# M2-TE/noetic-slam

Measured on AMD Instinct MI355X. Metric: scans/sec TSDF integration (128x1024 pts, 5 cm voxel), higher is better.
Workload: dtype f64+f32; 1 GPU; C1/M1 ouster_os1_128_1024x10_synthetic_5cm; global_batch=64, scans_per_gpu_batch=64, pipelined_batches=2, semantics=vdbfusion_f64, parallelism=single, front_end=two walks (k_count + k_place)

## Files before the change

### noetic-slam_amd/csrc/tsdf_capi.cpp

```cpp
#include <hip/hip_runtime.h>

#include <algorithm>
#include <array>
#include <atomic>
#include <cmath>
#include <cstdarg>
#include <cstddef>
#include <cstdio>
#include <cstdlib>
#include <cstring>
#include <numeric>
#include <chrono>
#include <condition_variable>
#include <functional>
#include <mutex>
#include <string>
#include <thread>
#include <utility>
#include <vector>

#include "../../include/tsdf_hip.h"
#include "../../include/tsdf_hip_raycast.h"
#include "../../include/tsdf_hip_sample.h"
#include "../../include/tsdf_mc_tables.h"
// ... 168 lines not shown
    H h = nullptr;
    HipHandle() = default;
    HipHandle(const HipHandle&) = delete;
    HipHandle& operator=(const HipHandle&) = delete;
    ~HipHandle() { if (h) (void)KILL(h); }
    hipError_t create() { return MAKE(&h, FLAGS); }
    operator H() const { return h; }
};
using Event = HipHandle<hipEvent_t, hipEventCreateWithFlags, hipEventDisableTiming, hipEventDestroy>;
using Stream = HipHandle<hipStream_t, hipStreamCreateWithFlags, hipStreamNonBlocking, hipStreamDestroy>;


struct Capacity {
    uint64_t max_bricks = 0, cap = 0;
    uint32_t max_active = 0;
    DevBuf<uint64_t> keys, brick_keys;
    DevBuf<uint32_t> slots, touched, cell[2];
    DevBuf<float> sdf, weight;
    DevBuf<uint4> active[2], active_ord[2], cagg[2];
};

struct Lane {
    DevBuf<uint32_t> pair, blk_n, plan, spn, ord_hist, act;
    DevBuf<uint4> blk, fb;
    DevBuf<uint2> smp;
    DevBuf<uint64_t> mg_ekey;
    DevBuf<uint32_t> mg_eidx, mg_bcnt, mg_bst, mg_bscan;
    DevBuf<float> mg_xyz, mg_w;
};

struct ScanRing {
    static constexpr int N = 16;
    PinBuf<ScanRec> host;
    DevBuf<ScanRec> dev;
    const ScanRec* host_dev = nullptr;
    PinBuf<unsigned long long> done;
    unsigned long long* done_dev = nullptr;
    Event ev[N];
    uint64_t next = 0;

    hipError_t create() {
        hipError_t e = host.alloc((size_t)N * (MAX_BATCH + 1));
        if (e == hipSuccess) e = dev.alloc((size_t)N * (MAX_BATCH + 1));
        void* dp = nullptr;
        if (e == hipSuccess) e = hipHostGetDevicePointer(&dp, host, 0);
        host_dev = static_cast<const ScanRec*>(dp);
// ... 5 lines not shown
        return e;
    }
};

}

struct tsdf_ctx {
    tsdf_params p{};
    int device = -1;
    Stream stream;
    RayConst R{};
    Table T{};
    Pool Pl{};
    Work W2[2]{};
    MgBufs mg[2];
    DevBuf<Globals> G;
    uint64_t max_points = 0;
    uint32_t max_batch = 0;
    CtxPlan plan;
    uint32_t max_fb = 0, max_smp = 0, max_spn = 0;
    int small_ns = 5;
    uint32_t count_wide = 512;
    bool count_paired = false;
    PinBuf<float> h_stage[2];
    Event stage_done[2];
    int stage_cur = 0;
    Stream bst[2];
    Capacity K;
    Lane lane[2];
    DevBuf<float> stage2[2];
    Event ev_main;
    Event ev_compact[2];
    hipEvent_t ev_integ[2] = {nullptr, nullptr};
    BatchDesc pend{};
    int pend_stage = 0;
    int last_stage = 1;
    uint64_t stage_reader[2] = {~0ull, ~0ull};
    Event stage_ev[2];
    ScanRing ring;
    HostTiming ht;
    uint64_t batch_id = 0;
    uint64_t n_scans = 0, n_batches = 0, n_points_in = 0;
    EventTimer* timer = nullptr;
    std::string err;
    struct Logged { uint64_t id; const float* xyz; BatchDesc D; };
    std::vector<Logged> log;
// ... 86 lines not shown
        if (rc) return rc;
    }
    D.s[0].blk = 0;
    for (uint32_t s = 0; s < D.n_scans; s++)
        D.s[s + 1].blk = D.s[s].blk + (D.s[s + 1].off - D.s[s].off + RPB - 1) / RPB;
    D.n_blocks = D.s[D.n_scans].blk;
    if (D.n_blocks > c->plan.max_blocks)
        return fail(c, TSDF_EINVAL, "batch needs %u workgroups > %u", D.n_blocks, c->plan.max_blocks);
    const int par = (int)(c->batch_id & 1);
    c->ht.lap(HT_PRE);
    const bool cross = c->p.pipeline != 0, lean = c->p.pipeline == 2;
    hipStream_t st = c->bst[cross ? par : 0];
    Table T = c->T;
    T.cell = c->K.cell[par];
    const Work& W = c->W2[par];
    const bool prev = cross && c->batch_id > 0;
    EventTimer* tm = c->timer;
    if (tm) tm->cur_batch = c->batch_id;
    if (c->metrics) c->metrics_info.push_back({c->batch_id, D.n_scans, D.s[D.n_scans].off});
    if (hipStreamQuery(c->stream) != hipSuccess) {
        HIPCHK(c, hipEventRecord(c->ev_main, c->stream));
        HIPCHK(c, hipStreamWaitEvent(st, c->ev_main, 0));
    }
    if (prev) HIPCHK(c, hipStreamWaitEvent(st, c->ev_compact[par ^ 1], 0));
    c->ht.lap(HT_WAITS);
    ScanRing& ring = c->ring;
    const uint64_t seq = ring.next++;
    const int slot = (int)(seq % ScanRing::N);
    if (const int rc = ring_wait(c, seq)) return rc;
    c->ht.lap(HT_RING_WAIT);
    const size_t at = (size_t)slot * (MAX_BATCH + 1);
    ScanRec* ds = ring.dev + at;
    std::memcpy(ring.host + at, D.s, (D.n_scans + 1) * sizeof(ScanRec));
    c->ht.lap(HT_RING_COPY);
    HIPCHK(c, launch_upload(ring.host_dev + at, ds, (uint32_t)((D.n_scans + 1) * sizeof(ScanRec)),
                            ring.done_dev, seq + 1, st));
    c->ht.lap(HT_UPLOAD);
    const BatchRef B{D.n_scans, D.n_blocks, ds};
    RayConst R = c->R;
    const float* d_rays = d_xyz;
    if (c->merged && D.n_blocks) {
        HIPCHK(c, launch_mg_prepass(d_xyz, B, D.n_blocks, D.s[D.n_scans].off, c->R, c->mg[par],
                                    &c->G->ctr[par].ovf, st));
        d_rays = c->mg[par].xyz_out;
        R.ray_w = c->mg[par].w_out;
    }
    const bool small = !c->plan.fused && D.n_scans <= (uint32_t)c->small_ns;
    const int k_front = c->plan.fused ? KIND_WALK : KIND_COUNT;
    const int k_back = c->plan.fused ? KIND_SPANS : KIND_PLACE;
    auto kt = [&](int kind) { return tm && !c->plan.fused && tm->want(kind) ? tm->timing(kind) : KTime{}; };
    if (D.n_blocks) {
        if (tm && c->plan.fused) tm->begin(k_front, st);
        if (c->R.sec_on) HIPCHK(c, launch_sector_flags(d_rays, B, R, W, c->G, par, st));
        if (c->plan.fused) HIPCHK(c, launch_walk(d_rays, B, R, T, W, c->G, par, c->plan.nstep, st));
        else HIPCHK(c, launch_count(d_rays, B, R, T, W, c->G, par, st, kt(KIND_COUNT),
                                    !c->R.sec_on && D.n_blocks <= c->count_wide,
                                    !c->R.sec_on && c->count_paired));
        c->ht.lap(HT_FRONT);
        if (tm && c->plan.fused) tm->next(k_front, KIND_COMPACT, st);
        HIPCHK(c, launch_compact(B, T, W, c->G, par, c->plan.fused, st, kt(KIND_COMPACT)));
        c->ht.lap(HT_COMPACT);
// ... 2 lines not shown
    if (prev && lean) HIPCHK(c, hipStreamWaitEvent(st, c->ev_integ[par ^ 1], 0));
    if (D.n_blocks) {
        if (tm && c->plan.fused) tm->next(KIND_COMPACT, k_back, st);
        if (c->plan.fused) HIPCHK(c, launch_spans(B, c->R, T, W, c->G, par, c->plan.nstep, st));
        else HIPCHK(c, launch_place(d_rays, B, R, T, W, c->G, par, st, kt(KIND_PLACE)));
        c->ht.lap(HT_BACK);
        if (tm && c->plan.fused) tm->end(k_back, st);
    }
    if (lean) HIPCHK(c, hipEventRecord(c->ev_compact[par], st));
    if (prev && !lean) HIPCHK(c, hipStreamWaitEvent(st, c->ev_integ[par ^ 1], 0));
    if (D.n_blocks) {
        if (tm && c->plan.fused) tm->begin(KIND_INTEGRATE, st);
        if (small) {
            HIPCHK(c, launch_integrate_small(B, c->R, T, W, c->Pl, c->G, par, st, kt(KIND_INTEGRATE)));
        } else {
            Work Wi = W;
            Wi.active = W.active_ord;
            HIPCHK(c, launch_integrate(B, c->R, T, Wi, c->Pl, c->G, par, c->plan.fused, c->max_batch > 64, st,
                                       kt(KIND_INTEGRATE)));
        }
        if (tm && c->plan.fused) tm->end(KIND_INTEGRATE, st);
        c->ht.lap(HT_INTEGRATE);
    }
    HIPCHK(c, launch_finish(c->G, par, (uint32_t)c->batch_id, st));
    if (cross) {
        HIPCHK(c, hipEventRecord(ring.ev[slot], st));
        c->ev_integ[par] = ring.ev[slot];
    }
    if (c->can_grow) c->log.push_back({c->batch_id, d_xyz, D});
    for (int k = 0; k < 2; k++)
        if (d_xyz == c->stage2[k]) {
            c->stage_reader[k] = c->batch_id;
            HIPCHK(c, hipEventRecord(c->stage_ev[k], st));
        }
    c->ht.lap(HT_FINISH);
    c->ht.n++;
    c->batch_id++;
    c->n_batches++;
    c->n_scans += D.n_scans;
    if (tm && tm->pending.size() > 8192) {
        HIPCHK(c, hipStreamSynchronize(c->bst[0]));
        HIPCHK(c, hipStreamSynchronize(c->bst[1]));
        tm->harvest();
    }
    return TSDF_OK;
}

// ... 238 lines not shown

static int emit_metrics(tsdf_ctx* c) {
    if (!c->metrics) return TSDF_OK;
    if (c->timer) c->timer->harvest();
    const uint64_t end = c->batch_id;
    if (end == c->metrics_next) return TSDF_OK;
    std::vector<BatchRecord> ring(METRIC_RING);
    HIPCHK(c, hipMemcpy(ring.data(), c->G->ring, sizeof(BatchRecord) * METRIC_RING,
                        hipMemcpyDeviceToHost));
    size_t ti = 0;
    for (uint64_t b = std::max<uint64_t>(c->metrics_next, end > METRIC_RING ? end - METRIC_RING : 0);
         b < end; b++) {
        const BatchRecord& r = ring[b % METRIC_RING];
        if (r.batch_id != (uint32_t)b) continue;
        uint32_t scans = 0;
        uint64_t points = 0;
        for (auto& i : c->metrics_info)
            if (i.id == b) { scans = i.scans; points = i.points; }
        const double bytes = 12.0 * (double)r.rays + 16.0 * (double)r.vox;
        fprintf(c->metrics,
                "{\"batch\": %llu, \"scans\": %u, \"points\": %llu, \"rays\": %llu, \"pairs\": %llu, "
                "\"voxel_updates\": %llu, \"dirty_voxels\": %llu, \"active_bricks\": %u, "
                "\"new_bricks\": %u, \"bricks\": %u, \"overflow\": %u, \"committed\": %s, "
                "\"algorithmic_bytes\": %.0f",
                (unsigned long long)b, scans, (unsigned long long)points,
                (unsigned long long)r.rays, (unsigned long long)r.pairs, (unsigned long long)r.vox,
                (unsigned long long)r.dirty, r.n_active, r.n_new,
                std::min<uint32_t>(r.pool_count, c->T.max_bricks), r.ovf,
                r.committed ? "true" : "false", bytes);
        const std::array<double, KIND_N>* ms = nullptr;
        if (c->timer) {
            auto& bm = c->timer->batch_ms;
            while (ti < bm.size() && bm[ti].first < b) ti++;
            if (ti < bm.size() && bm[ti].first == b) ms = &bm[ti].second;
        }
        if (ms) {
            double path = 0;
            for (int k = 0; k < KIND_N; k++) path += (*ms)[k];
            if (c->plan.fused)
                fprintf(c->metrics,
                        ", \"kernel_ms\": {\"walk\": %.5f, \"compact\": %.5f, \"spans\": %.5f, "
                        "\"integrate\": %.5f}",
                        (*ms)[KIND_WALK], (*ms)[KIND_COMPACT], (*ms)[KIND_SPANS], (*ms)[KIND_INTEGRATE]);
            else
                fprintf(c->metrics,
                        ", \"kernel_ms\": {\"count\": %.5f, \"compact\": %.5f, \"place\": %.5f, "
                        "\"integrate\": %.5f}",
                        (*ms)[KIND_COUNT], (*ms)[KIND_COMPACT], (*ms)[KIND_PLACE], (*ms)[KIND_INTEGRATE]);
            fprintf(c->metrics, ", \"path_ms\": %.5f, \"gbs\": %.2f", path,
                    path > 0 ? bytes / (path * 1e-3) / 1e9 : 0.0);
        }
        fprintf(c->metrics, "}\n");
// ... 204 lines not shown
    c->plan = ctx_plan(*p, PlanConsts{RPB, MAX_BATCH, WLK_THREADS, SPAN, VOX_LIMIT});
    if (!c->plan.refusal.empty()) return fail(c, TSDF_EINVAL, "%s", c->plan.refusal.c_str());
    c->R = ray_const(*p, c->plan.band_vox);
    c->merged = plan_merged(*p);
    c->idx_rule = p->n_sectors > 1 && p->sector_rule == TSDF_SECTOR_RULE_INDEX;
    c->max_points = p->max_points;
    c->max_batch = p->max_batch;
    c->max_fb = c->plan.max_fb;
    c->max_smp = c->plan.max_smp;
    c->max_spn = c->plan.max_spn;

    for (int q = 0; q < 2; q++) {
        Lane& L = c->lane[q];
        HIPCHK(c, L.pair.alloc(c->plan.fused ? 4 : c->plan.slots));
        HIPCHK(c, L.blk.alloc((size_t)c->plan.max_blocks * 2 * HCAP));
        HIPCHK(c, L.blk_n.alloc((size_t)c->plan.max_blocks * 2));
        HIPCHK(c, L.plan.alloc((size_t)c->plan.max_blocks * 2 * PLAN_STRIDE));
        HIPCHK(c, L.fb.alloc(c->max_fb));
        HIPCHK(c, L.smp.alloc_bytes((size_t)c->max_smp * smp_bytes(c->R.sem)));
        HIPCHK(c, L.spn.alloc(c->max_spn));
        HIPCHK(c, L.ord_hist.alloc(2 * 64 * 32));
        HIPCHK(c, hipMemset(L.ord_hist, 0, 2 * 64 * 32 * sizeof(uint32_t)));
        HIPCHK(c, L.act.alloc(c->plan.max_blocks));
        HIPCHK(c, c->stage2[q].alloc(c->plan.batch_points * 3));
        if (c->merged) {
            const uint64_t n = c->plan.batch_points, nb = mg_buckets_max(n);
            HIPCHK(c, L.mg_ekey.alloc(n));
            HIPCHK(c, L.mg_eidx.alloc(n));
            HIPCHK(c, L.mg_bcnt.alloc(MG_REPLICAS * nb));
            HIPCHK(c, hipMemset(L.mg_bcnt, 0, 4 * MG_REPLICAS * nb));
            HIPCHK(c, L.mg_bst.alloc(nb + 1));
            HIPCHK(c, L.mg_bscan.alloc(nb));
            HIPCHK(c, L.mg_xyz.alloc(n * 3));
            HIPCHK(c, L.mg_w.alloc(n));
        }
    }
    HIPCHK(c, c->G.alloc(1));
    if (const char* e = std::getenv("TSDF_SMALL_NS")) c->small_ns = std::max(0, std::min(8, std::atoi(e)));
    if (const char* e = std::getenv("TSDF_COUNT_WIDE")) c->count_wide = (uint32_t)std::max(0, std::atoi(e));
    if (const char* e = std::getenv("TSDF_COUNT_PAIRED")) c->count_paired = std::atoi(e) != 0;
    int nt = 4;
    if (const char* e = std::getenv("TSDF_PACK_THREADS")) nt = std::max(1, std::atoi(e));
    nt = std::min<int>(nt, (int)std::max(1u, std::thread::hardware_concurrency()));
    if (nt > 1) {
        try {
            c->pack = new PackPool(nt - 1);
        } catch (...) {
            c->pack = nullptr;
        }
    }
    HIPCHK(c, c->ring.create());
    HIPCHK(c, hipMemsetAsync(c->G, 0, sizeof(Globals), c->stream));
    Capacity K;
    if (const int rc = alloc_capacity(c, p->max_bricks, K)) return rc;
    HIPCHK(c, launch_fill(K.sdf, c->R.bg, p->max_bricks * BRICK_VOX, c->stream));
    HIPCHK(c, hipMemsetAsync(K.weight, 0, p->max_bricks * BRICK_VOX * sizeof(float), c->stream));
    c->K = std::move(K);
    set_views(c);
    for (int i = 0; i < 2; i++) {
        HIPCHK(c, c->h_stage[i].alloc(c->max_points * 3));
        HIPCHK(c, c->stage_done[i].create());
    }
    c->can_grow = p->max_bricks_hard == 0 || p->max_bricks_hard > p->max_bricks;
// ... 1617 lines not shown
```

### noetic-slam_amd/csrc/tsdf_device.h

```cpp
#pragma once
#include <hip/hip_ext.h>
#include <hip/hip_runtime.h>
#include <stdint.h>

namespace tsdf {

constexpr uint64_t EMPTY_KEY = ~0ull;
constexpr uint32_t UNASSIGNED = 0xFFFFFFFFu;
constexpr uint32_t INVALID_SLOT = 0xFFFFFFFEu;
constexpr uint32_t NO_PAIR = 0xFFFFFFFFu;
constexpr int BRICK_VOX = 512;
constexpr int BRICK_COORD_BIAS = 1 << 20;
constexpr int VOX_LIMIT = 1 << 23;
constexpr int MAX_DDA_STEPS = 1 << 20;
constexpr int MAX_BATCH = 512;
#ifndef TSDF_RPB
#define TSDF_RPB 1024
#endif
#ifndef TSDF_HCAP
#define TSDF_HCAP 2048
#endif
constexpr int RPB = TSDF_RPB;
constexpr int HCAP = TSDF_HCAP;
constexpr int LDS_PROBES = 64;
// ... 60 lines not shown
    if (!R.sec_on) return true;
    const float a = pseudo_angle(dx, dy);
    return R.sec_wrap ? (a >= R.sec_lo || a < R.sec_hi) : (a >= R.sec_lo && a < R.sec_hi);
}

struct ScanRec {
    uint32_t off, blk;
    float ox, oy, oz;
    float zx;
    double odx, ody, odz;
    float zy, zz;
    uint32_t xoff, pad;
};
static_assert(sizeof(ScanRec) == 64, "ScanRec layout");
struct BatchDesc {
    uint32_t n_scans;
    uint32_t n_blocks;
    ScanRec s[MAX_BATCH + 1];
};
struct BatchRef {
    uint32_t n_scans;
    uint32_t n_blocks;
    const ScanRec* __restrict__ s;
};

struct Table {
    uint64_t* keys;
    uint32_t* slots;
    uint32_t* touched;
    uint32_t* cell;
    uint64_t* brick_keys;
    uint64_t mask;
    uint32_t max_bricks;
    uint32_t cell_stride;
};

struct Pool {
    float* sdf;
    float* weight;
};

struct Work {
    uint32_t* pair;
    uint4* blk;
    uint32_t* blk_n;
    uint32_t* plan;
// ... 28 lines not shown
        return make_uint2(v.x, v.y);
    } else {
        return W.smp[i];
    }
}

struct Counters {
    uint32_t n_active;
    uint32_t cursor;
    uint32_t n_fb;
    uint32_t ovf;
    uint32_t n_new;
    uint32_t n_act;
    uint32_t pad1[2];
    unsigned long long n_vox[8];
    unsigned long long n_rays[8];
    unsigned long long n_pairs[8];
    unsigned long long n_dirty[8];
};

constexpr uint32_t METRIC_RING = 256;
struct BatchRecord {
    uint32_t batch_id, n_active, n_new, ovf;
    uint32_t committed, pool_count, pad[2];
    unsigned long long rays, pairs, vox, dirty;
};

struct Globals {
    uint32_t pool_count;
    uint32_t overflow;
    uint32_t failed;
    uint32_t retry;
    uint32_t fail_id;
    uint32_t pad[3];
    Counters ctr[2];
    unsigned long long tot_vox[8];
    unsigned long long tot_rays[8];
    unsigned long long tot_pairs[8];
    unsigned long long tot_dirty[8];
    Counters last;
    BatchRecord ring[METRIC_RING];
};

enum KernelKind {
    KIND_COUNT = 0, KIND_COMPACT = 1, KIND_PLACE = 2, KIND_INTEGRATE = 3,
    KIND_WALK = 4, KIND_SPANS = 5,
    KIND_N = 6
// ... 1 lines not shown

struct KTime {
    hipEvent_t start = nullptr, stop = nullptr;
};
template <typename... KArgs, typename... Args>
inline void tlaunch(void (*kern)(KArgs...), dim3 grid, dim3 block, hipStream_t st, hipEvent_t e0,
                    hipEvent_t e1, Args... args) {
    if (!e0 && !e1) {
        kern<<<grid, block, 0, st>>>(args...);
        return;
    }
    hipExtLaunchKernelGGL(kern, grid, block, 0, st, e0, e1, 0, args...);
}

struct KernelTimer {
    virtual void begin(int kind, hipStream_t st) = 0;
    virtual void end(int kind, hipStream_t st) = 0;
    virtual ~KernelTimer() {}
};

hipError_t launch_count(const float* d_xyz, const BatchRef& D, const RayConst& R, const Table& T,
                        const Work& Wk, Globals* G, int parity, hipStream_t st, const KTime& kt = {},
                        bool wide = false, bool paired = false);
#ifndef TSDF_CMP_CHUNK
#define TSDF_CMP_CHUNK 1024
#endif
constexpr uint32_t CMP_CHUNK = TSDF_CMP_CHUNK;
inline uint64_t compact_chunks(uint64_t cap) { return (cap + CMP_CHUNK - 1) / CMP_CHUNK; }
hipError_t launch_sector_flags(const float* d_xyz, const BatchRef& D, const RayConst& R,
                               const Work& Wk, Globals* G, int parity, hipStream_t st);
hipError_t launch_compact(const BatchRef& D, const Table& T, const Work& Wk, Globals* G,
                          int parity, bool fused, hipStream_t st, const KTime& kt = {});
hipError_t launch_walk(const float* d_xyz, const BatchRef& D, const RayConst& R, const Table& T,
                       const Work& Wk, Globals* G, int parity, int nstep, hipStream_t st);
hipError_t launch_spans(const BatchRef& D, const RayConst& R, const Table& T, const Work& Wk,
                        Globals* G, int parity, int nstep, hipStream_t st);
hipError_t launch_place(const float* d_xyz, const BatchRef& D, const RayConst& R, const Table& T,
                        const Work& Wk, Globals* G, int parity, hipStream_t st, const KTime& kt = {});
hipError_t launch_finish(Globals* G, int parity, uint32_t batch_id, hipStream_t st);
hipError_t launch_upload(const void* host_src, void* dst, uint32_t bytes,
                         unsigned long long* done, unsigned long long seq, hipStream_t st);
hipError_t launch_rehash(const Table& T, uint32_t n, Globals* G, hipStream_t st);
hipError_t launch_integrate_small(const BatchRef& D, const RayConst& R, const Table& T,
                                  const Work& Wk, const Pool& Pl, Globals* G, int parity,
                                  hipStream_t st, const KTime& kt = {});
hipError_t launch_integrate(const BatchRef& D, const RayConst& R, const Table& T, const Work& Wk,
                            const Pool& Pl, Globals* G, int parity, bool fused, bool big,
                            hipStream_t st, const KTime& kt = {});
hipError_t launch_query_dense(const Table& T, const Pool& Pl, const int64_t lo[3], const int dims[3],
                              float bg, float* d_sdf, float* d_w, hipStream_t st);
hipError_t launch_import(const Table& T, const Pool& Pl, const int32_t* d_coords, uint32_t n,
                         const float* d_sdf, const float* d_w, uint32_t* d_tidx, Globals* G,
                         float max_w, hipStream_t st);
hipError_t launch_fill(float* p, float v, uint64_t n, hipStream_t st);
constexpr int TILE_WORDS = 1028;
constexpr int MAX_WORLD = 64;
struct WorldCounts { uint64_t n[MAX_WORLD]; };
hipError_t launch_border_owner(const Table& T, uint32_t n_bricks, const uint64_t* d_all_keys,
                               const WorldCounts& counts, uint64_t stride, uint32_t rank,
                               uint32_t* d_owner, uint32_t* d_dest_n, hipStream_t st);
hipError_t launch_border_pack(const Table& T, const Pool& Pl, float bg, uint32_t n_bricks,
                              uint32_t rank, const uint32_t* d_owner, uint32_t* d_cursor,
// ... 76 lines not shown
```

### noetic-slam_amd/csrc/tsdf_kernels.hip

```cpp
#include <hip/hip_runtime.h>
#include <stdint.h>

#include <type_traits>

#include "tsdf_device.h"
#include "tsdf_ray.h"

namespace tsdf {


__device__ __forceinline__ uint32_t xcd_wedge(uint32_t p, uint32_t n, uint32_t G) {
    const uint32_t grp = 8u * G, g0 = p - p % grp;
    if (g0 + grp > n) return p;
    const uint32_t i = p - g0;
    return g0 + (i % 8u) * G + i / 8u;
}

__device__ __forceinline__ int lds_insert(unsigned long long* s_key, uint64_t key) {
    uint32_t hs = (uint32_t)(mix64(key) >> 40) & (HCAP - 1);
    for (int p = 0; p < LDS_PROBES; p++) {
        const unsigned long long k = s_key[hs];
        if (k == key) return (int)hs;
        if (k == EMPTY_KEY) {
            const unsigned long long old = atomicCAS(&s_key[hs], EMPTY_KEY, key);
// ... 39 lines not shown
    static_assert(G == 1 || RPB % NT == 0, "a pass over the rays stays inside one block");
    using CntT = typename std::conditional<G == 2, unsigned long long, uint32_t>::type;
    constexpr int PCAP = plan_cap(SEM), PW = plan_words(SEM);
    constexpr int NSUB = 2 * G;
    constexpr uint64_t KEY_G1 = 1ull << 63;
    __shared__ unsigned long long s_key[HCAP];
    __shared__ CntT s_cnt[HCAP];
    __shared__ unsigned long long red[2][NT / 64];
    __shared__ unsigned long long s_wsum[G][NT / 64];
    __shared__ uint32_t s_wcnt[G][NT / 64];
    __shared__ uint32_t s_bm[NSUB][PW];
    Counters* C = &G_->ctr[parity];
    uint32_t bx = xcd_wedge(blockIdx.x, gridDim.x, 16 / G);
    if constexpr (G == 1) {
        if (R.sec_on) {
            if (blockIdx.x >= C->n_act) return;
            bx = Wk.act[blockIdx.x];
        }
    }
#ifdef TSDF_CNT_PHASE
    unsigned long long cph[10] = {0, 0, 0, 0, 0, 0, 0, 0, 0, 0}, cpl = __builtin_readcyclecounter();
#endif
    uint32_t tb[G], r0b[G], r1b[G];
#pragma unroll
    for (int g = 0; g < G; g++) block_range(D, G * bx + g, tb[g], r0b[g], r1b[g]);
    const bool split = G == 2 && tb[G - 1] != tb[0];
    for (int j = threadIdx.x; j < HCAP; j += NT) {
        s_key[j] = EMPTY_KEY;
        s_cnt[j] = 0u;
    }
    for (int j = threadIdx.x; j < NSUB * PW; j += NT) (&s_bm[0][0])[j] = 0u;
    __syncthreads();
    CPH(0);
    const uint32_t maxp = Wk.maxp;
    uint32_t valid = 0, npairs = 0;
    auto pair_code = [&](uint64_t bkey, uint32_t cnt_in, uint32_t sub, uint32_t t) -> uint32_t {
        const uint64_t lkey = split && sub >= 2 ? bkey | KEY_G1 : bkey;
        const int lid = lds_insert(s_key, lkey);
        if (lid >= 0) {
            const CntT old = atomicAdd(&s_cnt[lid], (CntT)cnt_in << (16 * sub));
            const uint32_t lr = (uint32_t)(old >> (16 * sub)) & 0xFFFFu;
            return (cnt_in << PAIR_CNT_SHIFT) | ((uint32_t)lid << PAIR_LID_SHIFT) | lr;
        }
        const uint32_t f = atomicAdd(&C->n_fb, 1u);
        if (f >= Wk.max_fb) {
            atomicOr(&C->ovf, OVF_FB);
            return PAIR_DEAD;
        }
        const int64_t hx = table_insert(T, bkey, &C->ovf);
        if (hx < 0) return PAIR_DEAD;
        const uint32_t h = (uint32_t)hx;
        T.touched[h] = 1u;
        const uint32_t rk = atomicAdd(&T.cell[(size_t)h * T.cell_stride + t], cnt_in);
        Wk.fb[f] = make_uint4(h, t, rk, 0u);
        return PAIR_FB | (cnt_in << PAIR_CNT_SHIFT) | f;
    };
    constexpr int PASSES = G == 1 ? 1 : G * RPB / NT;
#pragma unroll 1
    for (int pass = 0; pass < PASSES; pass++) {
        const int g = G == 1 ? 0 : pass * NT / RPB;
        const uint32_t t = g ? tb[G - 1] : tb[0], r0 = g ? r0b[G - 1] : r0b[0];
        const uint32_t r1 = g ? r1b[G - 1] : r1b[0];
        const float ox = D.s[t].ox, oy = D.s[t].oy, oz = D.s[t].oz;
        const float* __restrict__ xs = scan_xyz(xyz, D, t, R);
        const uint32_t lo = G == 1 ? r0 + threadIdx.x : r0 + (uint32_t)(pass * NT) % RPB + threadIdx.x;
        const uint32_t hi = G == 1 ? r1 : min(r1, r0 + (uint32_t)(pass * NT) % RPB + NT);
        for (uint32_t i = lo; i < hi; i += NT) {
            uint32_t* pc = Wk.pair + (size_t)i * maxp;
            uint32_t k = 0;
            typename Walk<SEM>::State r;
            const bool ok = Walk<SEM>::init(R, D, t, i, xs[3 * (size_t)i], xs[3 * (size_t)i + 1],
                                            xs[3 * (size_t)i + 2], r);
            valid += ok ? 1u : 0u;
            const uint32_t sub = 2u * (uint32_t)g + (i - r0 >= (uint32_t)(RPB / 2) ? 1u : 0u);
            if (maxp <= 4) {
                uint64_t q0 = EMPTY_KEY, q1 = EMPTY_KEY, q2 = EMPTY_KEY, q3 = EMPTY_KEY;
                uint32_t n0 = 0, n1 = 0, n2 = 0, n3 = 0, np = 0;
#ifdef TSDF_ABLATE_CNT_NOWALK
                if (ok && r.px == 1e30f) {
#else
                if (ok) {
#endif
                    const int bx0 = r.vx >> 3, by0 = r.vy >> 3, bz0 = r.vz >> 3;
                    uint32_t c0 = 0, c1 = 0, c2 = 0, c3 = 0, curc = ~0u, ccount = 0;
                    auto walk = [&](auto chk) {
                        for (int it = 0; it < MAX_DDA_STEPS; it++) {
                            const bool gt = Walk<SEM>::gate_sel(R, ox, oy, oz, r, decltype(chk)::value);
                            const uint32_t bc = brick_code_of(r.vx, r.vy, r.vz);
                            const bool nb = gt && bc != curc;
                            const bool cl = nb && curc != ~0u;
                            c0 = (cl && np == 0) ? curc : c0; n0 = (cl && np == 0) ? ccount : n0;
                            c1 = (cl && np == 1) ? curc : c1; n1 = (cl && np == 1) ? ccount : n1;
                            c2 = (cl && np == 2) ? curc : c2; n2 = (cl && np == 2) ? ccount : n2;
                            c3 = (cl && np == 3) ? curc : c3; n3 = (cl && np == 3) ? ccount : n3;
                            np += cl ? 1u : 0u;
                            curc = nb ? bc : curc;
                            ccount = (nb ? 0u : ccount) + (gt ? 1u : 0u);
// ... 257 lines not shown
                                                             BatchRef D, RayConst R, Work Wk,
                                                             Globals* G, int parity) {
    const uint32_t b = blockIdx.x * (FLG_THREADS / 64) + (threadIdx.x >> 6);
    if (b >= D.n_blocks) return;
    uint32_t t, r0, r1;
    block_range(D, b, t, r0, r1);
    const float ox = D.s[t].ox, oy = D.s[t].oy;
    const float* __restrict__ xs = scan_xyz(xyz, D, t, R);
    bool any = false;
    for (uint32_t i = r0 + (threadIdx.x & 63); i < r1; i += 64)
        any |= in_sector(R, xs[3 * (size_t)i] - ox, xs[3 * (size_t)i + 1] - oy);
    const bool v = __any(any);
    if ((threadIdx.x & 63) == 0 && v) Wk.act[atomicAdd(&G->ctr[parity].n_act, 1u)] = b;
}

hipError_t launch_sector_flags(const float* d_xyz, const BatchRef& D, const RayConst& R,
                               const Work& Wk, Globals* G, int parity, hipStream_t st) {
    const uint32_t per = FLG_THREADS / 64;
    k_sector_flags<<<(D.n_blocks + per - 1) / per, FLG_THREADS, 0, st>>>(d_xyz, D, R, Wk, G,
                                                                        parity);
    return hipGetLastError();
}


constexpr int ORD_BLOCKS = 64;
constexpr int ORD_CLASSES = 32;

__device__ __forceinline__ uint32_t size_class(uint32_t n) {
    return (uint32_t)__clz(max(n, 1u));
}
__device__ __forceinline__ uint32_t ord_chunk_slice(uint32_t c, uint32_t nch) {
    return (uint32_t)(((uint64_t)c * ORD_BLOCKS) / nch);
}


constexpr int CMP_THREADS = 256;
constexpr int CMP_PER = CMP_CHUNK / CMP_THREADS;
constexpr int CMP_GROUP = 16;
constexpr int CMP_SCAN_THREADS = 1024;

template <int NT>
__device__ __forceinline__ uint32_t block_excl_scan(uint32_t x, uint32_t* s_w, uint32_t* total) {
    constexpr int NW = NT / 64;
    const int lane = threadIdx.x & 63, wid = threadIdx.x >> 6;
    const uint32_t v = wave_incl_scan(x);
    if (lane == 63) s_w[wid] = v;
// ... 296 lines not shown
                                                      const Globals* __restrict__ G, int parity) {
    constexpr int STG = plan_cap(SEM), PW = plan_words(SEM);
    __shared__ uint32_t s_base[HCAP];
    __shared__ uint16_t s_loff[HCAP];
    __shared__ uint16_t s_ord[HCAP];
    __shared__ uint32_t s_bits[PW];
    __shared__ uint16_t s_wpre[(PW + 1) & ~1];
    __shared__ float st_s[STG];
    typedef typename std::conditional<SEM == 3, uint32_t, uint16_t>::type StL;
    __shared__ StL st_l[STG];
    __shared__ float s_w0[SEM == 3 ? PLC_THREADS : 1];
    __shared__ uint32_t s_vote[2][PLC_THREADS / 64];
#ifdef TSDF_PLC_PHASE
    unsigned long long pt[6];
    if (threadIdx.x == 0) pt[0] = clock64();
#endif
    uint32_t wb = xcd_wedge(blockIdx.x, gridDim.x, 32);
    if (R.sec_on) {
        if ((blockIdx.x >> 1) >= G->ctr[parity].n_act) return;
        wb = 2 * Wk.act[blockIdx.x >> 1] + (blockIdx.x & 1u);
    }
    uint32_t t, r0, r1;
    block_range(D, wb >> 1, t, r0, r1);
    r0 += (wb & 1u) * PLC_THREADS;
    const uint4* bt = Wk.blk + (size_t)wb * HCAP;
    const uint32_t maxp = Wk.maxp;
    const uint32_t i = r0 + threadIdx.x;
    float px = 0.0f, py = 0.0f, pz = 0.0f;
    uint4 code4 = make_uint4(NO_PAIR, NO_PAIR, NO_PAIR, NO_PAIR);
    const uint32_t* pc = Wk.pair + (size_t)i * maxp;
    if (i < r1) {
        const float* __restrict__ xs = scan_xyz(xyz, D, t, R);
        px = xs[3 * (size_t)i];
        py = xs[3 * (size_t)i + 1];
        pz = xs[3 * (size_t)i + 2];
        if (maxp == 4) code4 = *reinterpret_cast<const uint4*>(pc);
    }
    const uint32_t nruns = Wk.blk_n[wb];
    static_assert(PLC_THREADS <= HCAP, "a lane's first list entry lies inside the list");
    const uint4 e0 = bt[threadIdx.x];
    const uint32_t* pl = Wk.plan + (size_t)wb * PLAN_STRIDE;
    static_assert(PW <= PLC_THREADS, "one bitmap word per lane");
    const uint32_t plan_bits = threadIdx.x < (uint32_t)PW ? pl[threadIdx.x] : 0u;
    const uint32_t plan_pre =
        threadIdx.x < (uint32_t)((PW + 1) / 2) ? pl[PW + threadIdx.x] : 0u;
    const uint32_t plan_nst = pl[PLAN_STRIDE - 1];
    const bool late = maxp <= 4;
    const uint32_t cell0 = (threadIdx.x < nruns && e0.x != NO_PAIR)
                               ? T.cell[(size_t)e0.x * T.cell_stride + t]
                               : NO_PAIR;
    const float ox = D.s[t].ox, oy = D.s[t].oy, oz = D.s[t].oz;
    typename Walk<SEM>::State r;
    const bool ok = i < r1 && Walk<SEM>::init(R, D, t, i, px, py, pz, r);
    if (R.sec_on && !block_any<PLC_THREADS>(ok, s_vote[0])) return;
    if constexpr (SEM == 3) s_w0[threadIdx.x] = ok ? r.w0 : 0.0f;
    if (threadIdx.x < (uint32_t)PW) s_bits[threadIdx.x] = plan_bits;
    if (threadIdx.x < (uint32_t)((PW + 1) / 2))
        reinterpret_cast<uint32_t*>(s_wpre)[threadIdx.x] = plan_pre;
#ifdef TSDF_PLC_PHASE
    if (threadIdx.x == 0) pt[1] = clock64();
#endif
    auto fill = [&](uint32_t j, const uint4& e) {
        const uint32_t slot = e.w >> 16;
        const bool stg = e.z < (uint32_t)STG;
        s_loff[slot] = stg ? (uint16_t)e.z : (uint16_t)0xFFFFu;
        if (stg) s_ord[j] = (uint16_t)slot;
    };
    auto run_base = [&](const uint4& e, uint32_t cell) {
        return e.x != NO_PAIR ? cell + e.y : NO_PAIR;
    };
    if (threadIdx.x < nruns) {
        fill(threadIdx.x, e0);
        if (!late) s_base[e0.w >> 16] = run_base(e0, cell0);
    }
    for (uint32_t j = threadIdx.x + PLC_THREADS; j < nruns; j += PLC_THREADS) {
        const uint4 e = bt[j];
// ... 286 lines not shown
        tlaunch(k, D.n_blocks, CNT_THREADS, st, kt.start, kt.stop, d_xyz, D, R, T, Wk, G, parity);
    }
    return hipGetLastError();
}

hipError_t launch_compact(const BatchRef& D, const Table& T, const Work& Wk, Globals* G,
                          int parity, bool fused, hipStream_t st, const KTime& kt) {
    const uint32_t nch = (uint32_t)compact_chunks(T.mask + 1);
    tlaunch(fused ? k_compact_sum<true> : k_compact_sum<false>, nch, CMP_THREADS, st, kt.start,
            nullptr, D.n_scans, T, Wk);
    k_compact_scan<<<1, CMP_SCAN_THREADS, 0, st>>>(nch, Wk, G, parity, fused ? 1 : 0);
    tlaunch(fused ? k_compact_write<true> : k_compact_write<false>, nch, CMP_THREADS, st, nullptr,
            kt.stop, D.n_scans, nch, T, Wk, G, parity);
    return hipGetLastError();
}

hipError_t launch_place(const float* d_xyz, const BatchRef& D, const RayConst& R, const Table& T,
                        const Work& Wk, Globals* G, int parity, hipStream_t st, const KTime& kt) {
    auto k = R.sem == 1 ? k_place<1> : R.sem == 3 ? k_place<3> : R.sem == 2 ? k_place<2> : k_place<0>;
    tlaunch(k, 2 * D.n_blocks, PLC_THREADS, st, kt.start, kt.stop, d_xyz, D, R, T, Wk, G, parity);
    return hipGetLastError();
}

__global__ void k_finish(Globals* G, int parity, uint32_t batch_id) {
    constexpr int NW = sizeof(Counters) / 4;
    Counters* C = &G->ctr[parity];
    const uint32_t ovf = C->ovf, failed = G->failed;
    const bool commit = !(G->retry && (ovf || failed));
    __syncthreads();
    if (threadIdx.x < 8 && commit) {
        const int k = threadIdx.x;
        G->tot_rays[k] += C->n_rays[k];
        G->tot_pairs[k] += C->n_pairs[k];
        G->tot_vox[k] += C->n_vox[k];
        G->tot_dirty[k] += C->n_dirty[k];
    }
    if (threadIdx.x == 0 && ovf) {
        G->overflow |= ovf;
        if (!failed) {
            G->failed = 1u;
            G->fail_id = batch_id;
        }
    }
    if (threadIdx.x == 0) {
        BatchRecord r;
        r.batch_id = batch_id;
        r.n_active = C->n_active;
        r.n_new = C->n_new;
        r.ovf = ovf;
        r.committed = commit ? 1u : 0u;
        r.pool_count = G->pool_count;
        r.pad[0] = r.pad[1] = 0u;
        r.rays = r.pairs = r.vox = r.dirty = 0ull;
        for (int k = 0; k < 8; k++) {
            r.rays += C->n_rays[k];
            r.pairs += C->n_pairs[k];
            r.vox += C->n_vox[k];
            r.dirty += C->n_dirty[k];
        }
        G->ring[batch_id % METRIC_RING] = r;
    }
    __syncthreads();
    uint32_t* src = reinterpret_cast<uint32_t*>(C);
    uint32_t* dst = reinterpret_cast<uint32_t*>(&G->last);
    for (int j = threadIdx.x; j < NW; j += blockDim.x) {
        dst[j] = src[j];
        src[j] = 0u;
    }
}

__global__ void k_upload(const uint4* __restrict__ src, uint4* __restrict__ dst, uint32_t n,
                         unsigned long long* done, unsigned long long seq) {
    for (uint32_t i = threadIdx.x; i < n; i += blockDim.x) dst[i] = src[i];
    __syncthreads();
    if (threadIdx.x == 0)
        __hip_atomic_fetch_max(done, seq, __ATOMIC_RELEASE, __HIP_MEMORY_SCOPE_SYSTEM);
}

hipError_t launch_upload(const void* host_src, void* dst, uint32_t bytes,
                         unsigned long long* done, unsigned long long seq, hipStream_t st) {
    k_upload<<<1, 256, 0, st>>>(static_cast<const uint4*>(host_src), static_cast<uint4*>(dst),
                                bytes / 16, done, seq);
    return hipGetLastError();
}

hipError_t launch_finish(Globals* G, int parity, uint32_t batch_id, hipStream_t st) {
    k_finish<<<1, 64, 0, st>>>(G, parity, batch_id);
    return hipGetLastError();
}

__global__ void k_rehash(Table T, uint32_t n, Globals* G) {
    for (uint32_t slot = blockIdx.x * blockDim.x + threadIdx.x; slot < n;
         slot += gridDim.x * blockDim.x) {
        const int64_t h = table_insert(T, T.brick_keys[slot], &G->overflow);
        if (h >= 0) T.slots[h] = slot;
    }
}

hipError_t launch_rehash(const Table& T, uint32_t n, Globals* G, hipStream_t st) {
    if (n) k_rehash<<<grid_for(n, 256, 4096), 256, 0, st>>>(T, n, G);
    return hipGetLastError();
}

hipError_t launch_query_dense(const Table& T, const Pool& Pl, const int64_t lo[3], const int dims[3],
                              float bg, float* d_sdf, float* d_w, hipStream_t st) {
    const uint64_t total = (uint64_t)dims[0] * dims[1] * dims[2];
    k_query_dense<<<grid_for(total, 256, 8192), 256, 0, st>>>(T, Pl, lo[0], lo[1], lo[2], dims[0],
                                                              dims[1], dims[2], bg, d_sdf, d_w);
    return hipGetLastError();
}
// ... 27 lines not shown
```

### noetic-slam_amd/csrc/tsdf_ray.h

```cpp
#pragma once
#include <hip/hip_runtime.h>
#include <stdint.h>

#include "tsdf_device.h"

namespace tsdf {



constexpr float FAR_LIMIT = 1073741824.0f;

__device__ __forceinline__ bool far_ok(float x, float y, float z) {
    return __builtin_fabsf(x) < FAR_LIMIT && __builtin_fabsf(y) < FAR_LIMIT &&
           __builtin_fabsf(z) < FAR_LIMIT;
}

__device__ __forceinline__ bool start_inside(int vx, int vy, int vz, int band_vox) {
    const int lim = VOX_LIMIT - band_vox;
    return vx > -lim && vx < lim && vy > -lim && vy < lim && vz > -lim && vz < lim;
}

struct RayState {
    float px, py, pz;
    float t1i;
    float tnx, tny, tnz;
    float tdx, tdy, tdz;
// ... 141 lines not shown
    const float t = mx ? r.tnx : (my ? r.tny : r.tnz);
    const bool adv = t <= r.t1i;
    r.tnx = (mx && adv) ? r.tnx + r.tdx : r.tnx;
    r.tny = (my && adv) ? r.tny + r.tdy : r.tny;
    r.tnz = (mz && adv) ? r.tnz + r.tdz : r.tnz;
    r.vx += (mx && adv) ? r.sx : 0;
    r.vy += (my && adv) ? r.sy : 0;
    r.vz += (mz && adv) ? r.sz : 0;
    return adv;
}


__device__ __forceinline__ void block_range(const BatchRef& D, uint32_t b, uint32_t& t,
                                            uint32_t& r0, uint32_t& r1) {
    uint32_t lo = 0, hi = D.n_scans;
    while (hi - lo > 1) {
        const uint32_t mid = (lo + hi) >> 1;
        if (D.s[mid].blk <= b) lo = mid;
        else hi = mid;
    }
    t = lo;
    r0 = D.s[t].off + (b - D.s[t].blk) * RPB;
    r1 = min(D.s[t + 1].off, r0 + RPB);
}

__device__ __forceinline__ const float* scan_xyz(const float* xyz, const BatchRef& D, uint32_t t,
                                                 const RayConst& R) {
    return R.ray_w ? xyz : xyz + 3 * (size_t)D.s[t].xoff;
}

constexpr float VB_MIN_WEIGHT = 1.0f / 65536.0f;

struct VbState {
    float px;
    float dx, dy, dz;
    float depth;
    float tnx, tny, tnz;
    float tdx, tdy, tdz;
    int vx, vy, vz;
    int sx, sy, sz;
    int rem;
    float w0;
};

__device__ __forceinline__ void vb_axis(float ss, float es, int& v, int& st, float& tn, float& td,
                                        int& steps) {
// ... 528 lines not shown
```

Before: 60170 scans/s.

## Remap rays to 32x32 column-beam tiles in count and place walks

Adds per-scan detection of the column-major organized-scan height and remaps each workgroup's 1024 rays to a 32-column by 32-beam tile instead of a contiguous run. Spatially compact tiles should touch fewer distinct bricks per workgroup, shrinking the shared hash tables and brick runs produced by k_count and k_place. It costs an extra detection kernel per batch, strided point loads, and a per-batch tiled-scan counter in the finish kernel. The ray-to-block mapping is no longer contiguous, and the detection relies on elevation-monotonicity heuristics.

```diff
diff --git a/noetic-slam_amd/csrc/ray_tile.h b/noetic-slam_amd/csrc/ray_tile.h
--- /dev/null
+++ b/noetic-slam_amd/csrc/ray_tile.h
@@ -0,0 +1,88 @@
+#pragma once
+#include <math.h>
+#include <stdint.h>
+
+#if defined(__HIPCC__) || defined(__CUDACC__)
+#define RAY_TILE_HD __host__ __device__
+#else
+#define RAY_TILE_HD
+#endif
+
+namespace tsdf {
+
+constexpr uint32_t TILE_RAYS = 1024;
+constexpr uint32_t TILE_COLS = 32;
+constexpr uint32_t TILE_BEAMS = 32;
+#ifndef TSDF_TILE_HALF_BEAMS
+#define TSDF_TILE_HALF_BEAMS 16
+#endif
+constexpr uint32_t TILE_HALF_BEAMS = TSDF_TILE_HALF_BEAMS;
+static_assert(TILE_HALF_BEAMS == 16 || TILE_HALF_BEAMS == 32, "a half is half a block's tile");
+
+RAY_TILE_HD inline bool tile_height_ok(uint32_t H) {
+    return H == 0 || (H % TILE_BEAMS == 0 && H >= 64 && H <= 256);
+}
+
+struct TileBlock {
+    uint32_t base, H;
+};
+
+RAY_TILE_HD inline TileBlock tile_block(uint32_t n, uint32_t H, uint32_t b) {
+    if (H != 0) {
+        const uint32_t bpg = H / TILE_BEAMS, g = b / bpg, G = TILE_COLS * H;
+        if ((uint64_t)(g + 1) * G <= n) return TileBlock{g * G + TILE_BEAMS * (b - g * bpg), H};
+    }
+    return TileBlock{b * TILE_RAYS, 0u};
+}
+
+RAY_TILE_HD inline uint32_t tile_point(const TileBlock& tb, uint32_t s) {
+    if (tb.H == 0) return tb.base + s;
+    const uint32_t hf = s >> 9, q = s & 511u;
+    const uint32_t c = TILE_HALF_BEAMS == 16 ? q >> 4 : 16u * hf + (q >> 5);
+    const uint32_t bm = TILE_HALF_BEAMS == 16 ? 16u * hf + (q & 15u) : q & 31u;
+    return tb.base + c * tb.H + bm;
+}
+
+
+RAY_TILE_HD inline float tile_elev(const float* p, float ox, float oy, float oz) {
+    const float dx = p[0] - ox, dy = p[1] - oy, dz = p[2] - oz;
+    return dz / sqrtf(dx * dx + dy * dy);
+}
+
+RAY_TILE_HD inline bool tile_boundary_ok(const float* xyz, uint32_t H, uint32_t c, float ox,
+                                         float oy, float oz, float dir) {
+    const float* p = xyz + 3 * (size_t)(c * H - 2);
+    const float e0 = tile_elev(p, ox, oy, oz), e1 = tile_elev(p + 3, ox, oy, oz);
+    const float e2 = tile_elev(p + 6, ox, oy, oz), e3 = tile_elev(p + 9, ox, oy, oz);
+    const float* m = xyz + 3 * (size_t)(c * H + H / 2 - 1);
+    const float m0 = tile_elev(m, ox, oy, oz), m1 = tile_elev(m + 3, ox, oy, oz);
+    return dir * (e1 - e0) > 0.0f && dir * (e2 - e1) < 0.0f && dir * (e3 - e2) > 0.0f &&
+           dir * (m1 - m0) > 0.0f;
+}
+
+RAY_TILE_HD inline float tile_direction(const float* xyz, uint32_t H, float ox, float oy,
+                                        float oz) {
+    const float d0 = tile_elev(xyz + 3, ox, oy, oz) - tile_elev(xyz, ox, oy, oz);
+    const float* m = xyz + 3 * (size_t)(H / 2 - 1);
+    const float d1 = tile_elev(m + 3, ox, oy, oz) - tile_elev(m, ox, oy, oz);
+    if (d0 > 0.0f && d1 > 0.0f) return 1.0f;
+    if (d0 < 0.0f && d1 < 0.0f) return -1.0f;
+    return 0.0f;
+}
+
+RAY_TILE_HD inline bool tile_shape_ok(uint32_t n, uint32_t H) {
+    return H >= 64 && n % H == 0 && n / H >= 2;
+}
+
+inline uint32_t tile_detect(const float* xyz, uint32_t n, float ox, float oy, float oz) {
+    for (uint32_t H = 64; H <= 256; H *= 2) {
+        if (!tile_shape_ok(n, H)) continue;
+        const float dir = tile_direction(xyz, H, ox, oy, oz);
+        bool ok = dir != 0.0f;
+        for (uint32_t c = 1; ok && c < n / H; c++) ok = tile_boundary_ok(xyz, H, c, ox, oy, oz, dir);
+        if (ok) return H;
+    }
+    return 0u;
+}
+
+}
diff --git a/noetic-slam_amd/csrc/tsdf_capi.cpp b/noetic-slam_amd/csrc/tsdf_capi.cpp
--- a/noetic-slam_amd/csrc/tsdf_capi.cpp
+++ b/noetic-slam_amd/csrc/tsdf_capi.cpp
@@ -214,6 +214,7 @@
 
 struct Lane {
     DevBuf<uint32_t> pair, blk_n, plan, spn, ord_hist, act;
+    DevBuf<uint32_t> tile;
     DevBuf<uint4> blk, fb;
     DevBuf<uint2> smp;
     DevBuf<uint64_t> mg_ekey;
@@ -265,6 +266,7 @@
     int small_ns = 5;
     uint32_t count_wide = 512;
     bool count_paired = false;
+    int ray_tiles = -1;
     PinBuf<float> h_stage[2];
     Event stage_done[2];
     int stage_cur = 0;
@@ -397,8 +399,6 @@
         HIPCHK(c, hipEventRecord(c->ev_main, c->stream));
         HIPCHK(c, hipStreamWaitEvent(st, c->ev_main, 0));
     }
-    if (prev) HIPCHK(c, hipStreamWaitEvent(st, c->ev_compact[par ^ 1], 0));
-    c->ht.lap(HT_WAITS);
     ScanRing& ring = c->ring;
     const uint64_t seq = ring.next++;
     const int slot = (int)(seq % ScanRing::N);
@@ -408,10 +408,18 @@
     ScanRec* ds = ring.dev + at;
     std::memcpy(ring.host + at, D.s, (D.n_scans + 1) * sizeof(ScanRec));
     c->ht.lap(HT_RING_COPY);
+    const bool tiles = c->ray_tiles != 0 && !c->R.sec_on && !c->idx_rule && !c->merged &&
+                       !c->plan.fused && D.n_blocks != 0;
+    uint32_t* const d_tile = tiles ? c->lane[par].tile.p : nullptr;
+    if (tiles)
+        HIPCHK(c, launch_tile_detect(d_xyz, BatchRef{D.n_scans, D.n_blocks, ring.host_dev + at, nullptr},
+                                     d_tile, c->ray_tiles > 0 ? (uint32_t)c->ray_tiles : 0u, st));
+    if (prev) HIPCHK(c, hipStreamWaitEvent(st, c->ev_compact[par ^ 1], 0));
+    c->ht.lap(HT_WAITS);
     HIPCHK(c, launch_upload(ring.host_dev + at, ds, (uint32_t)((D.n_scans + 1) * sizeof(ScanRec)),
                             ring.done_dev, seq + 1, st));
     c->ht.lap(HT_UPLOAD);
-    const BatchRef B{D.n_scans, D.n_blocks, ds};
+    const BatchRef B{D.n_scans, D.n_blocks, ds, d_tile};
     RayConst R = c->R;
     const float* d_rays = d_xyz;
     if (c->merged && D.n_blocks) {
@@ -460,7 +468,7 @@
         if (tm && c->plan.fused) tm->end(KIND_INTEGRATE, st);
         c->ht.lap(HT_INTEGRATE);
     }
-    HIPCHK(c, launch_finish(c->G, par, (uint32_t)c->batch_id, st));
+    HIPCHK(c, launch_finish(c->G, par, (uint32_t)c->batch_id, B, st));
     if (cross) {
         HIPCHK(c, hipEventRecord(ring.ev[slot], st));
         c->ev_integ[par] = ring.ev[slot];
@@ -745,12 +753,12 @@
                 "{\"batch\": %llu, \"scans\": %u, \"points\": %llu, \"rays\": %llu, \"pairs\": %llu, "
                 "\"voxel_updates\": %llu, \"dirty_voxels\": %llu, \"active_bricks\": %u, "
                 "\"new_bricks\": %u, \"bricks\": %u, \"overflow\": %u, \"committed\": %s, "
-                "\"algorithmic_bytes\": %.0f",
+                "\"tiled_scans\": %u, \"algorithmic_bytes\": %.0f",
                 (unsigned long long)b, scans, (unsigned long long)points,
                 (unsigned long long)r.rays, (unsigned long long)r.pairs, (unsigned long long)r.vox,
                 (unsigned long long)r.dirty, r.n_active, r.n_new,
                 std::min<uint32_t>(r.pool_count, c->T.max_bricks), r.ovf,
-                r.committed ? "true" : "false", bytes);
+                r.committed ? "true" : "false", r.tiled, bytes);
         const std::array<double, KIND_N>* ms = nullptr;
         if (c->timer) {
             auto& bm = c->timer->batch_ms;
@@ -1001,6 +1009,7 @@
         HIPCHK(c, L.ord_hist.alloc(2 * 64 * 32));
         HIPCHK(c, hipMemset(L.ord_hist, 0, 2 * 64 * 32 * sizeof(uint32_t)));
         HIPCHK(c, L.act.alloc(c->plan.max_blocks));
+        HIPCHK(c, L.tile.alloc(c->max_batch));
         HIPCHK(c, c->stage2[q].alloc(c->plan.batch_points * 3));
         if (c->merged) {
             const uint64_t n = c->plan.batch_points, nb = mg_buckets_max(n);
@@ -1018,6 +1027,10 @@
     if (const char* e = std::getenv("TSDF_SMALL_NS")) c->small_ns = std::max(0, std::min(8, std::atoi(e)));
     if (const char* e = std::getenv("TSDF_COUNT_WIDE")) c->count_wide = (uint32_t)std::max(0, std::atoi(e));
     if (const char* e = std::getenv("TSDF_COUNT_PAIRED")) c->count_paired = std::atoi(e) != 0;
+    if (const char* e = std::getenv("TSDF_RAY_TILES")) {
+        const int h = std::atoi(e);
+        c->ray_tiles = h == 64 || h == 128 || h == 256 ? h : 0;
+    }
     int nt = 4;
     if (const char* e = std::getenv("TSDF_PACK_THREADS")) nt = std::max(1, std::atoi(e));
     nt = std::min<int>(nt, (int)std::max(1u, std::thread::hardware_concurrency()));
diff --git a/noetic-slam_amd/csrc/tsdf_device.h b/noetic-slam_amd/csrc/tsdf_device.h
--- a/noetic-slam_amd/csrc/tsdf_device.h
+++ b/noetic-slam_amd/csrc/tsdf_device.h
@@ -106,6 +106,7 @@
     uint32_t n_scans;
     uint32_t n_blocks;
     const ScanRec* __restrict__ s;
+    const uint32_t* __restrict__ tile;
 };
 
 struct Table {
@@ -180,7 +181,9 @@
 constexpr uint32_t METRIC_RING = 256;
 struct BatchRecord {
     uint32_t batch_id, n_active, n_new, ovf;
-    uint32_t committed, pool_count, pad[2];
+    uint32_t committed, pool_count;
+    uint32_t tiled;
+    uint32_t pad;
     unsigned long long rays, pairs, vox, dirty;
 };
 
@@ -228,6 +231,8 @@
 hipError_t launch_count(const float* d_xyz, const BatchRef& D, const RayConst& R, const Table& T,
                         const Work& Wk, Globals* G, int parity, hipStream_t st, const KTime& kt = {},
                         bool wide = false, bool paired = false);
+hipError_t launch_tile_detect(const float* d_xyz, const BatchRef& D, uint32_t* tile,
+                              uint32_t force, hipStream_t st);
 #ifndef TSDF_CMP_CHUNK
 #define TSDF_CMP_CHUNK 1024
 #endif
@@ -243,7 +248,8 @@
                         Globals* G, int parity, int nstep, hipStream_t st);
 hipError_t launch_place(const float* d_xyz, const BatchRef& D, const RayConst& R, const Table& T,
                         const Work& Wk, Globals* G, int parity, hipStream_t st, const KTime& kt = {});
-hipError_t launch_finish(Globals* G, int parity, uint32_t batch_id, hipStream_t st);
+hipError_t launch_finish(Globals* G, int parity, uint32_t batch_id, const BatchRef& D,
+                         hipStream_t st);
 hipError_t launch_upload(const void* host_src, void* dst, uint32_t bytes,
                          unsigned long long* done, unsigned long long seq, hipStream_t st);
 hipError_t launch_rehash(const Table& T, uint32_t n, Globals* G, hipStream_t st);
diff --git a/noetic-slam_amd/csrc/tsdf_kernels.hip b/noetic-slam_amd/csrc/tsdf_kernels.hip
--- a/noetic-slam_amd/csrc/tsdf_kernels.hip
+++ b/noetic-slam_amd/csrc/tsdf_kernels.hip
@@ -85,8 +85,12 @@
     unsigned long long cph[10] = {0, 0, 0, 0, 0, 0, 0, 0, 0, 0}, cpl = __builtin_readcyclecounter();
 #endif
     uint32_t tb[G], r0b[G], r1b[G];
-#pragma unroll
-    for (int g = 0; g < G; g++) block_range(D, G * bx + g, tb[g], r0b[g], r1b[g]);
+    TileBlock tlb[G];
+#pragma unroll
+    for (int g = 0; g < G; g++) {
+        block_range(D, G * bx + g, tb[g], r0b[g], r1b[g]);
+        tlb[g] = block_tile(D, G * bx + g, tb[g]);
+    }
     const bool split = G == 2 && tb[G - 1] != tb[0];
     for (int j = threadIdx.x; j < HCAP; j += NT) {
         s_key[j] = EMPTY_KEY;
@@ -126,16 +130,19 @@
         const uint32_t r1 = g ? r1b[G - 1] : r1b[0];
         const float ox = D.s[t].ox, oy = D.s[t].oy, oz = D.s[t].oz;
         const float* __restrict__ xs = scan_xyz(xyz, D, t, R);
-        const uint32_t lo = G == 1 ? r0 + threadIdx.x : r0 + (uint32_t)(pass * NT) % RPB + threadIdx.x;
-        const uint32_t hi = G == 1 ? r1 : min(r1, r0 + (uint32_t)(pass * NT) % RPB + NT);
-        for (uint32_t i = lo; i < hi; i += NT) {
+        const TileBlock tl = g ? tlb[G - 1] : tlb[0];
+        const uint32_t ray0 = D.s[t].off, nsl = r1 > r0 ? r1 - r0 : 0u;
+        const uint32_t lo = G == 1 ? threadIdx.x : (uint32_t)(pass * NT) % RPB + threadIdx.x;
+        const uint32_t hi = G == 1 ? nsl : min(nsl, (uint32_t)(pass * NT) % RPB + NT);
+        for (uint32_t sl = lo; sl < hi; sl += NT) {
+            const uint32_t i = ray0 + tile_point(tl, sl);
             uint32_t* pc = Wk.pair + (size_t)i * maxp;
             uint32_t k = 0;
             typename Walk<SEM>::State r;
             const bool ok = Walk<SEM>::init(R, D, t, i, xs[3 * (size_t)i], xs[3 * (size_t)i + 1],
                                             xs[3 * (size_t)i + 2], r);
             valid += ok ? 1u : 0u;
-            const uint32_t sub = 2u * (uint32_t)g + (i - r0 >= (uint32_t)(RPB / 2) ? 1u : 0u);
+            const uint32_t sub = 2u * (uint32_t)g + (sl >= (uint32_t)(RPB / 2) ? 1u : 0u);
             if (maxp <= 4) {
                 uint64_t q0 = EMPTY_KEY, q1 = EMPTY_KEY, q2 = EMPTY_KEY, q3 = EMPTY_KEY;
                 uint32_t n0 = 0, n1 = 0, n2 = 0, n3 = 0, np = 0;
@@ -439,6 +446,37 @@
     return hipGetLastError();
 }
 
+constexpr int TDT_THREADS = 1024;
+__global__ __launch_bounds__(TDT_THREADS) void k_tile_detect(const float* __restrict__ xyz,
+                                                            BatchRef D, uint32_t* __restrict__ tile,
+                                                            uint32_t force) {
+    const uint32_t t = blockIdx.x;
+    if (force) {
+        if (threadIdx.x == 0) tile[t] = force;
+        return;
+    }
+    const uint32_t n = D.s[t + 1].off - D.s[t].off;
+    const float* __restrict__ xs = xyz + 3 * ((size_t)D.s[t].off + D.s[t].xoff);
+    const float ox = D.s[t].ox, oy = D.s[t].oy, oz = D.s[t].oz;
+    uint32_t found = 0;
+    for (uint32_t H = 64; H <= 256 && !found; H *= 2) {
+        if (!tile_shape_ok(n, H)) continue;
+        const float dir = tile_direction(xs, H, ox, oy, oz);
+        bool ok = dir != 0.0f && tile_boundary_ok(xs, H, 1, ox, oy, oz, dir);
+        if (ok)
+            for (uint32_t c = 2 + threadIdx.x; ok && c < n / H; c += TDT_THREADS)
+                ok = tile_boundary_ok(xs, H, c, ox, oy, oz, dir);
+        if (__syncthreads_and(ok)) found = H;
+    }
+    if (threadIdx.x == 0) tile[t] = found;
+}
+
+hipError_t launch_tile_detect(const float* d_xyz, const BatchRef& D, uint32_t* tile,
+                              uint32_t force, hipStream_t st) {
+    k_tile_detect<<<D.n_scans, TDT_THREADS, 0, st>>>(d_xyz, D, tile, force);
+    return hipGetLastError();
+}
+
 
 constexpr int ORD_BLOCKS = 64;
 constexpr int ORD_CLASSES = 32;
@@ -781,14 +819,15 @@
     }
     uint32_t t, r0, r1;
     block_range(D, wb >> 1, t, r0, r1);
-    r0 += (wb & 1u) * PLC_THREADS;
+    const uint32_t sl = (wb & 1u) * PLC_THREADS + threadIdx.x;
+    const bool has_ray = r0 + sl < r1;
+    const uint32_t i = D.s[t].off + tile_point(block_tile(D, wb >> 1, t), sl);
     const uint4* bt = Wk.blk + (size_t)wb * HCAP;
     const uint32_t maxp = Wk.maxp;
-    const uint32_t i = r0 + threadIdx.x;
     float px = 0.0f, py = 0.0f, pz = 0.0f;
     uint4 code4 = make_uint4(NO_PAIR, NO_PAIR, NO_PAIR, NO_PAIR);
     const uint32_t* pc = Wk.pair + (size_t)i * maxp;
-    if (i < r1) {
+    if (has_ray) {
         const float* __restrict__ xs = scan_xyz(xyz, D, t, R);
         px = xs[3 * (size_t)i];
         py = xs[3 * (size_t)i + 1];
@@ -810,7 +849,7 @@
                                : NO_PAIR;
     const float ox = D.s[t].ox, oy = D.s[t].oy, oz = D.s[t].oz;
     typename Walk<SEM>::State r;
-    const bool ok = i < r1 && Walk<SEM>::init(R, D, t, i, px, py, pz, r);
+    const bool ok = has_ray && Walk<SEM>::init(R, D, t, i, px, py, pz, r);
     if (R.sec_on && !block_any<PLC_THREADS>(ok, s_vote[0])) return;
     if constexpr (SEM == 3) s_w0[threadIdx.x] = ok ? r.w0 : 0.0f;
     if (threadIdx.x < (uint32_t)PW) s_bits[threadIdx.x] = plan_bits;
@@ -1143,10 +1182,15 @@
     return hipGetLastError();
 }
 
-__global__ void k_finish(Globals* G, int parity, uint32_t batch_id) {
+__global__ void k_finish(Globals* G, int parity, uint32_t batch_id,
+                         const uint32_t* __restrict__ tile, uint32_t n_scans) {
     constexpr int NW = sizeof(Counters) / 4;
     Counters* C = &G->ctr[parity];
     const uint32_t ovf = C->ovf, failed = G->failed;
+    uint32_t tiled = 0;
+    if (tile)
+        for (uint32_t j = threadIdx.x; j < n_scans; j += 64) tiled += tile[j] ? 1u : 0u;
+    tiled = wave_sum<uint32_t>(tiled);
     const bool commit = !(G->retry && (ovf || failed));
     __syncthreads();
     if (threadIdx.x < 8 && commit) {
@@ -1171,7 +1215,8 @@
         r.ovf = ovf;
         r.committed = commit ? 1u : 0u;
         r.pool_count = G->pool_count;
-        r.pad[0] = r.pad[1] = 0u;
+        r.tiled = tiled;
+        r.pad = 0u;
         r.rays = r.pairs = r.vox = r.dirty = 0ull;
         for (int k = 0; k < 8; k++) {
             r.rays += C->n_rays[k];
@@ -1205,8 +1250,9 @@
     return hipGetLastError();
 }
 
-hipError_t launch_finish(Globals* G, int parity, uint32_t batch_id, hipStream_t st) {
-    k_finish<<<1, 64, 0, st>>>(G, parity, batch_id);
+hipError_t launch_finish(Globals* G, int parity, uint32_t batch_id, const BatchRef& D,
+                         hipStream_t st) {
+    k_finish<<<1, 64, 0, st>>>(G, parity, batch_id, D.tile, D.n_scans);
     return hipGetLastError();
 }
 
diff --git a/noetic-slam_amd/csrc/tsdf_ray.h b/noetic-slam_amd/csrc/tsdf_ray.h
--- a/noetic-slam_amd/csrc/tsdf_ray.h
+++ b/noetic-slam_amd/csrc/tsdf_ray.h
@@ -2,6 +2,7 @@
 #include <hip/hip_runtime.h>
 #include <stdint.h>
 
+#include "ray_tile.h"
 #include "tsdf_device.h"
 
 namespace tsdf {
@@ -189,6 +190,12 @@
     t = lo;
     r0 = D.s[t].off + (b - D.s[t].blk) * RPB;
     r1 = min(D.s[t + 1].off, r0 + RPB);
+}
+
+static_assert(RPB == (int)TILE_RAYS, "ray_tile.h maps blocks of RPB slots");
+__device__ __forceinline__ TileBlock block_tile(const BatchRef& D, uint32_t b, uint32_t t) {
+    const uint32_t H = D.tile ? D.tile[t] : 0u;
+    return tile_block(D.s[t + 1].off - D.s[t].off, H, b - D.s[t].blk);
 }
 
 __device__ __forceinline__ const float* scan_xyz(const float* xyz, const BatchRef& D, uint32_t t,
diff --git a/profiles/ray_tiles/run_count.py b/profiles/ray_tiles/run_count.py
--- /dev/null
+++ b/profiles/ray_tiles/run_count.py
@@ -0,0 +1,58 @@
+import argparse
+import os
+import sys
+
+import numpy as np
+
+REPO = os.path.dirname(os.path.dirname(os.path.dirname(os.path.abspath(__file__))))
+sys.path.insert(0, os.path.join(REPO, "noetic-slam_amd"))
+
+VS, TAU, H = 0.05, 0.15, 128
+
+
+def brick_ids(pts, org):
+    d = pts.astype(np.float64) - org
+    u = d / np.linalg.norm(d, axis=1, keepdims=True)
+    s = np.linspace(-TAU, TAU, 25)
+    pos = pts[:, None, :].astype(np.float64) + s[None, :, None] * u[:, None, :]
+    b = np.floor(pos / (8 * VS)).astype(np.int64) + (1 << 20)
+    return (b[..., 0] << 42) | (b[..., 1] << 21) | b[..., 2]
+
+
+def unit_of(n, cols, beams):
+    i = np.arange(n)
+    c, b = i // H, i % H
+    return (c // cols) * (H // beams) + b // beams
+
+
+def runs(bricks, unit):
+    key = np.stack([np.broadcast_to(unit[:, None], bricks.shape).ravel(), bricks.ravel()], 1)
+    return np.unique(key, axis=0).shape[0]
+
+
+def main():
+    ap = argparse.ArgumentParser()
+    ap.add_argument("--scans", type=int, nargs="+", default=[0, 300, 700])
+    ap.add_argument("--drop", type=float, default=0.0)
+    a = ap.parse_args()
+    from tsdf_map.scan_gen import OusterSim
+    sim = OusterSim()
+    layouts = [("k_count block", 8, 128), ("k_count block", 32, 32), ("k_count block", 64, 16),
+               ("k_count 2048", 16, 128),
+               ("k_place half", 4, 128), ("k_place half", 16, 32), ("k_place half", 32, 16)]
+    tot = {l: 0 for l in layouts}
+    rng = np.random.default_rng(1)
+    for k in a.scans:
+        pts, org = sim.scan(k)
+        if a.drop > 0:
+            pts = pts[rng.random(pts.shape[0]) >= a.drop]
+        br = brick_ids(pts, org)
+        for l in layouts:
+            tot[l] += runs(br, unit_of(pts.shape[0], l[1], l[2]))
+    print("scans %s, drop %g: runs per scan" % (a.scans, a.drop))
+    for l in layouts:
+        print("  %-14s %3d x %3d  %8.1f k" % (l[0], l[1], l[2], tot[l] / len(a.scans) / 1e3))
+
+
+if __name__ == "__main__":
+    main()
```

New measurement: 61390 scans/s (median of 6 runs). +2.0%, better.
